# cassiusfive/balatro-gym

Hardware: AMD Instinct MI355X
Metric: env-steps/sec at 65536 envs, random policy; achieved HBM GB/s vs peak (higher is better)
Workload: dtype int64/f64

## Files before the change

### balatro_gym_amd/csrc/bg_device.h

```cpp
#pragma once
#include <hip/hip_runtime.h>
#include <stdint.h>
#include "bg_tables.h"

#define BG_NHOT 8
#define BG_NDECK 4
#define BG_NCOLD 7
#define BG_NTMPL 2
#define BG_MT_N 624
#define BG_MT_M 397
#define BG_MTS 640
#define BG_BLOCK 64

#define BG_DEVERR_GSTREAM 1u
#define BG_DEVERR_SHOPBLK 2u
#define BG_DEVERR_DECKRING 4u
#define BG_DEVERR_SHOPRING 8u

typedef __attribute__((address_space(1))) unsigned long long g_u64;
typedef __attribute__((address_space(1))) uint32_t g_u32;
__device__ __forceinline__ unsigned long long bg_ld8a(const void* p) { return __hip_atomic_load((g_u64*)p, __ATOMIC_RELAXED, __HIP_MEMORY_SCOPE_AGENT); }
__device__ __forceinline__ uint32_t bg_ld4a(const void* p) { return __hip_atomic_load((g_u32*)p, __ATOMIC_RELAXED, __HIP_MEMORY_SCOPE_AGENT); }
__device__ __forceinline__ void bg_st8a(void* p, unsigned long long v) { __hip_atomic_store((g_u64*)p, v, __ATOMIC_RELAXED, __HIP_MEMORY_SCOPE_AGENT); }
__device__ __forceinline__ uint4 bg_ld16a(const void* p) {
// ... 202 lines not shown
}
__device__ __forceinline__ Deck0 bg_load_deck0(const BgDev& d, int env) {
  uint4 c = d.deck[env];
  Deck0 r;
  r.lo = ((uint64_t)c.y << 32) | c.x;
  r.hi = ((uint64_t)c.w << 32) | c.z;
  return r;
}
__device__ __forceinline__ void bg_deck_set(Deck0& dk, int k, uint4 c) {
  if (k == 0) { dk.lo = ((uint64_t)c.y << 32) | c.x; dk.hi = ((uint64_t)c.w << 32) | c.z; }
}
__device__ __forceinline__ void bg_deck_set(DeckLds& dk, int k, uint4 c) {
  dk.col[(4 * k) * BG_RB] = c.x; dk.col[(4 * k + 1) * BG_RB] = c.y; dk.col[(4 * k + 2) * BG_RB] = c.z; dk.col[(4 * k + 3) * BG_RB] = c.w;
}
__device__ __forceinline__ int bg_card(const BgDev& d, int env, const Deck0& k, int idx) {
  if (idx < 16) return (int)(((idx < 8 ? k.lo : k.hi) >> (8 * (idx & 7))) & 0xffull);
  const uint32_t* p = (const uint32_t*)&d.deck[(size_t)(idx >> 4) * d.N + env];
  return (int)((bg_ld4a(p + ((idx & 15) >> 2)) >> (8 * (idx & 3))) & 0xffu);
}
template <int S, bool C> struct DeckLdsS { lds_u32* col; static constexpr bool kCards = C; };
template <int S, bool C>
__device__ __forceinline__ void bg_deck_set(DeckLdsS<S, C>& dk, int k, uint4 c) {
  dk.col[(4 * k) * S] = c.x; dk.col[(4 * k + 1) * S] = c.y; dk.col[(4 * k + 2) * S] = c.z; dk.col[(4 * k + 3) * S] = c.w;
}
template <int S, bool C>
__device__ __forceinline__ int bg_card(const BgDev& d, int env, const DeckLdsS<S, C>& k, int idx) {
  return (int)((const lds_u8*)k.col)[(idx >> 2) * (S * 4) + (idx & 3)];
}
__device__ __forceinline__ int bg_card(const BgDev& d, int env, const DeckLds& k, int idx) {
  return (int)((const lds_u8*)k.col)[(idx >> 2) * (BG_RB * 4) + (idx & 3)];
}

struct DeckHead { uint64_t lo, hi; };
__device__ __forceinline__ DeckHead bg_deck_head(const BgDev& d, int env, const Deck0& k) { return DeckHead{k.lo, k.hi}; }
template <int S, bool C>
__device__ __forceinline__ DeckHead bg_deck_head(const BgDev& d, int env, const DeckLdsS<S, C>& k) {
  const uint32_t a = k.col[0], b = k.col[S], c = k.col[2 * S], e = k.col[3 * S];
  return DeckHead{((uint64_t)b << 32) | a, ((uint64_t)e << 32) | c};
}
template <class DK>
__device__ __forceinline__ int bg_card_h(const BgDev& d, int env, const DK& k, const DeckHead& h, int idx) {
  if (idx < 16) return (int)(((idx < 8 ? h.lo : h.hi) >> (8 * (idx & 7))) & 0xffull);
  return bg_card(d, env, k, idx);
}

__device__ __forceinline__ uint32_t bg_temper(uint32_t y) {
  y ^= (y >> 11);
  y ^= (y << 7) & 0x9d2c5680u;
  y ^= (y << 15) & 0xefc60000u;
  y ^= (y >> 18);
  return y;
}
__device__ __forceinline__ uint32_t bg_twist(uint32_t a, uint32_t b, uint32_t far) {
  uint32_t y = (a & 0x80000000u) | (b & 0x7fffffffu);
  return far ^ (y >> 1) ^ ((y & 1u) ? 0x9908b0dfu : 0u);
}

// ... 300 lines not shown
```

### balatro_gym_amd/csrc/bg_engine3.h

```cpp
#pragma once

#ifdef BG_E3_TIMING
#define E3T_DECL() unsigned long long e3t_[8] = {0,0,0,0,0,0,0,0}, e3t0_ = __builtin_readcyclecounter()
#define E3T(k) do { const unsigned long long n_ = __builtin_readcyclecounter(); e3t_[k] += n_ - e3t0_; e3t0_ = n_; } while (0)
#define E3T_CNT(k, v) do { e3t_[k] += (v); } while (0)
#define E3T_FLUSH(base) do { if (lane == 0 && d.dbg) for (int k_ = 0; k_ < 8; k_++) atomicAdd(&d.dbg[(base) + k_], e3t_[k_]); } while (0)
constexpr bool kE3Timing = true, kE3Tl = true;
#else
#define E3T_DECL() const unsigned long long e3t_[8] = {0,0,0,0,0,0,0,0}; (void)e3t_
#define E3T(k) do {} while (0)
#define E3T_CNT(k, v) do {} while (0)
#define E3T_FLUSH(base) do {} while (0)
constexpr bool kE3Timing = false;
#ifdef BG_E3_TL
constexpr bool kE3Tl = true;
#else
constexpr bool kE3Tl = false;
#endif
#endif

#define BG_E3_REC_STORE(v, p) __builtin_nontemporal_store(v, p)
#define BG_E3_SPARSE 8u
#define BG_E3_SPARSE2 16u
#define BG_E3_ACTB 8
template <int NOW, int KS, int NSV>
struct E3Lds {
  static constexpr int NE = NOW * KS * BG_BLOCK;
  bg_u32x4 s_img[NE][22];
  uint4 s_c34[2][NE];
  unsigned long long s_mask[NE];
  uint32_t s_prod[NE];
  uint16_t s_ans[NE];
  uint32_t s_q[2][NE];
  __attribute__((aligned(16))) uint32_t s_ctl[8];
  uint32_t s_win[NSV][BG_WIN][BG_BLOCK];
  uint2 s_list[NOW][KS * BG_BLOCK];
  uint4 s_nd[BG_NDECK][NE];
  uint32_t s_ndst[NE];
  bg_u32x4 s_zero;
  unsigned long long s_stats[6];
  uint32_t s_owners_left;
  JTables jt;
};
template <bool HASH, bool CARDS, int NOW, int KS, int NSV, bool ACT = false>
__global__ __launch_bounds__((NOW + NSV) * BG_BLOCK, 2) void bg_engine3_kernel(BgDev d, EngineArgs a) {
  constexpr int NE = NOW * KS * BG_BLOCK, LNE = NE == 256 ? 8 : (NE == 128 ? 7 : 6);
  static_assert(NE == 64 || NE == 128 || NE == 256, "envs per workgroup (a request carries the env's lane in 8 bits)");
  __shared__ E3Lds<NOW, KS, NSV> L;
  auto& s_img = L.s_img; auto& s_c34 = L.s_c34; auto& s_mask = L.s_mask; auto& s_prod = L.s_prod; auto& s_ans = L.s_ans; auto& s_q = L.s_q;
  auto& s_ctl = L.s_ctl; auto& s_win = L.s_win; auto& s_list = L.s_list; auto& s_zero = L.s_zero; auto& s_owners_left = L.s_owners_left; auto& jt = L.jt;
  auto& s_nd = L.s_nd; auto& s_ndst = L.s_ndst;
  __shared__ int s_actb[ACT ? BG_E3_ACTB : 1][ACT ? NE : 1];
  __builtin_amdgcn_s_setprio(2);
  const unsigned long long e3_k0 = kE3Tl ? wall_clock64() : 0ull;
  BG_PROBE_INIT();
  bg_tables_load(&jt, d.jtab);
  const int tid = threadIdx.x, lane = tid & 63;
  const int wave = tid >> 6;
  const int epw = (NE == 64 && a.epw >= 1u && a.epw < 64u) ? (int)a.epw : NE;
  const int env0 = blockIdx.x * epw;
  const int n_live = d.N - env0 < epw ? d.N - env0 : epw;
  using DeckT = typename std::conditional<CARDS, Deck0C, Deck0>::type;
  const size_t N = (size_t)d.N;
  typedef __attribute__((address_space(3))) const char lds_cc;
  if (tid < 8) s_ctl[tid] = 0;
  if (tid == 0) { s_zero = bg_u32x4{0u, 0u, 0u, 0u}; s_owners_left = NOW; }
  if (tid < 6) L.s_stats[tid] = 0ull;
  for (int l = tid; l < NE; l += (NOW + NSV) * BG_BLOCK) {
    const int env = env0 + l;
    s_q[0][l] = 0; s_q[1][l] = 0; s_ans[l] = 0; s_ndst[l] = 0;
    if (l < n_live) {
      uint4 c[BG_NHOT];
#pragma unroll
      for (int k = 0; k < BG_NHOT; k++) c[k] = d.hot[(size_t)k * N + env];
      s_c34[0][l] = c[3]; s_c34[1][l] = c[4];
      DeckT dk; static_cast<Deck0&>(dk) = bg_load_deck0(d, env);
      const uint32_t prod = d.prod_view ? d.prod_view[env] : 0u;
      s_prod[l] = prod;
      Env e;
      bg_unpack(c, e);
      bg_derive_ready(e, prod);
      s_ndst[l] = e.d_ready > 0 ? 1u : 0u;
      if (e.d_ready > 0) {
#pragma unroll
        for (int k = 0; k < BG_NDECK; k++) s_nd[k][l] = d.ndeck[((size_t)e.d_head * BG_NDECK + k) * N + env];
      }
      ShopRegs sr; sr.valid = false;
      const uint64_t mask = bg_action_mask(d, env, e, sr);
      s_mask[l] = mask;
      const ObsPtrs none{};
      bg_write_obs_impl<false, 3>(d, env, 0, e, dk, none, mask, sr, RowExtra{0.0, 0, 0u}, RowStage{(lds_u4*)&s_img[l][0], nullptr});
    }
  }
  __syncthreads();
  if constexpr (kE3Timing) if (lane == 0) { uint32_t hw; asm volatile("s_getreg_b32 %0, hwreg(HW_REG_HW_ID)" : "=s"(hw)); atomicOr(&s_ctl[2], ((hw >> 4) & 3u) << (2 * wave)); }
  const unsigned long long e3_w0 = kE3Tl ? wall_clock64() : 0ull;
  if constexpr (kE3Tl) {
    if (tid == 0 && d.dbg) atomicAdd(&d.dbg[28], e3_w0 - e3_k0);
    __syncthreads();
  }
  const uint32_t T = (uint32_t)a.T;
  if (wave < NOW) {
    const uint32_t bmod3 = (uint32_t)(a.env_index0 % 3ull);
    lds_cc* const imgb = (lds_cc*)&s_img[0][0];
    const bool whole = a.obs.row_stride == 384u;
    uint32_t rsel[3], cmul[3], cib[3], cgl[3];
#pragma unroll
    for (int j = 0; j < 3; j++) {
      const uint32_t pidx = (uint32_t)j * BG_BLOCK + (uint32_t)lane, rs = (pidx * 2731u) >> 16, c = pidx - 24u * rs;
      rsel[j] = rs; cgl[j] = 16u * c;
      cmul[j] = c < 22u ? 16u * 22u : 0u;
      cib[j] = c < 22u ? 16u * c : (uint32_t)((lds_cc*)&s_zero - imgb);
    }
    uint32_t t[KS], nreq[KS];
    bool waiting[KS], terminal[KS];
    uint4 rc3[KS], rc4[KS];
    uint64_t rmask[KS];
    uint64_t px[KS];
    size_t prow[KS];
    int pblind[KS];
    uint32_t abase[KS];
    uint32_t athr[KS];
#pragma unroll
    for (int s = 0; s < KS; s++) {
      t[s] = 0; nreq[s] = 0; waiting[s] = false;
      const int l = (wave * KS + s) * BG_BLOCK + lane;
      if constexpr (ACT) {
        abase[s] = 0; athr[s] = 100u;
        prow[s] = (size_t)(env0 + l);
        if (l < n_live) {
          const uint32_t cap = (d.hot[(size_t)7 * N + (size_t)(env0 + l)].w >> 16) & 0xffu;
          if (cap > 0u && cap < 100u) athr[s] = cap;
        }
      } else {
        const int env = env0 + l;
        const uint64_t gi0 = a.env_index0 + (uint64_t)env;
        px[s] = a.policy_seed + 0x9E3779B97F4A7C15ull * (gi0 + 1) + BG_POLICY_PSI * (a.t0 + 1);
        prow[s] = (size_t)env;
        pblind[s] = a.policy == 2 ? 45 + (int)((bmod3 + (uint32_t)env % 3u) % 3u) : 45;
      }
      rc3[s] = s_c34[0][l]; rc4[s] = s_c34[1][l]; rmask[s] = s_mask[l];
      const lds_u32* im = (const lds_u32*)&s_img[l][0];
      terminal[s] = bg_b(rc3[s].x, 0) > (ACT ? athr[s] : 100u) || (int64_t)(((uint64_t)im[33] << 32) | im[32]) > 1000000000ll;
    }
    uint64_t n_steps = 0, rbits = 0, ohash = 0;
    uint32_t idle = 0, aiter = 0;
    E3T_DECL();
    for (;;) {
      bg_u32x4 ndv[KS][BG_NDECK];
      bool ndp[KS];
#pragma unroll
      for (int s = 0; s < KS; s++) ndp[s] = false;
      bool busy = false;
#pragma unroll
      for (int s = 0; s < KS; s++) busy = busy || ((wave * KS + s) * BG_BLOCK + lane < n_live && (t[s] < T || waiting[s]));
      if (__ballot(busy) == 0ull) break;
      E3T_CNT(4, 1);
      if constexpr (ACT) {
// ... 21 lines not shown
        const int l = (wave * KS + s) * BG_BLOCK + lane, env = env0 + l;
        const bool live = l < n_live;
        lds_u32* const img32 = (lds_u32*)&s_img[l][0];
        lds_u8* const img8 = (lds_u8*)&s_img[l][0];
        const size_t row = prow[s];
        bool fin = false;
        if (waiting[s] && bg_lds_ld(&s_ans[l]) == (nreq[s] & 0xffffu)) {
          waiting[s] = false; fin = true;
          const uint32_t nds = bg_lds_ld(&s_ndst[l]);
          if ((nds & 0xffu) == 2u) {
#pragma unroll
            for (int k = 0; k < BG_NDECK; k++) ndv[s][k] = *(const __attribute__((address_space(1))) bg_u32x4*)&d.ndeck[((size_t)(nds >> 8) * BG_NDECK + k) * N + env];
            bg_lds_st(&s_ndst[l], 0u);
            ndp[s] = true;
          }
          rc3[s] = s_c34[0][l]; rc4[s] = s_c34[1][l]; rmask[s] = s_mask[l];
          terminal[s] = bg_b(rc3[s].x, 0) > (ACT ? athr[s] : 100u) || (int64_t)(((uint64_t)img32[33] << 32) | img32[32]) > 1000000000ll;
        }
        else if (live && !waiting[s] && t[s] < T) {
          uint64_t mask = rmask[s];
          const uint4 c3 = rc3[s];
          const uint32_t phase = bg_b(c3.x, 2), discards_left = bg_b(c3.y, 0), nsel0 = bg_b(c3.y, 3);
          int action;
          if constexpr (ACT) action = s_actb[(t[s] - abase[s]) & (BG_E3_ACTB - 1u)][l];
          else {
            Env pe; pe.phase = (int)phase;
            PolicyLane pl; pl.seed_env = 0; pl.blind = pblind[s];
            action = bg_policy_action_fast(pe, mask, a.policy, pl, px[s], (lds_JTables*)&jt);
          }
          double reward = 0.0;
          const bool valid = action >= 0 && action < 60 && ((mask >> (action & 63)) & 1ull);
          const bool term = terminal[s];
          if (!term && valid && phase == 0u && action >= 2 && action < 10) {
            const int pos = action - 2;
            Env te; te.sel = ((uint64_t)rc4[s].w << 32) | rc4[s].z; te.nsel = (int)nsel0;
            bg_toggle_select(te, pos);
            rc4[s].z = (uint32_t)te.sel; rc4[s].w = (uint32_t)(te.sel >> 32);
            rc3[s].y = (rc3[s].y & 0x00ffffffu) | ((uint32_t)te.nsel << 24);
            *(lds_u64*)&img32[2 * pos] = te.nsel > (int)nsel0 ? 1ull : 0ull;
            if ((te.nsel > 0) != (nsel0 > 0u)) {
              const uint32_t play = te.nsel > 0 ? 1u : 0u, disc = (te.nsel > 0 && discards_left > 0u) ? 1u : 0u;
              mask = (mask & ~3ull) | play | ((uint64_t)disc << 1);
              rmask[s] = mask;
              *(__attribute__((address_space(3))) uint16_t*)&img8[BG_ROW_ACTION_MASK] = (uint16_t)(play | (disc << 8));
            }
            fin = true;
          } else if (!term && valid && phase == 1u && action == 31 && (int)(int8_t)bg_b(c3.y, 1) <= (int)bg_b(c3.y, 2)) {
            const uint32_t nhand = bg_b(c3.y, 2), ncons = bg_b(c3.z, 1);
            rc3[s].x &= 0xff00ffffu;
            uint64_t m = (((1ull << (nhand < 8u ? nhand : 8u)) - 1ull) << 2) | (((1ull << ncons) - 1ull) << 10);
            if (nsel0 > 0u) m |= 1ull | (discards_left > 0u ? 2ull : 0ull);
            mask = m;
            rmask[s] = mask;
#pragma unroll
            for (int wq = 0; wq < 15; wq++) img32[44 + wq] = __umul24((uint32_t)(mask >> (4 * wq)) & 0xfu, 0x204081u) & 0x01010101u;
#pragma unroll
            for (int wq = 64; wq < 74; wq++) img32[wq] = 0u;
            img8[BG_ROW_PHASE] = 0;
            fin = true;
          } else if (!term && !valid) { reward = -1.0; fin = true; }
          else {
            s_c34[0][l] = rc3[s]; s_c34[1][l] = rc4[s]; s_mask[l] = mask;
            if constexpr (ACT) img32[43] = (uint32_t)action;
            const int q = (!term && phase == 0u && action == 0) ? 0 : 1;
            const uint32_t slot = __hip_atomic_fetch_add(&s_ctl[q], 1u, __ATOMIC_RELAXED, __HIP_MEMORY_SCOPE_WORKGROUP);
            bg_lds_st(&s_q[q][slot & (NE - 1)], (uint32_t)l | (((slot >> LNE) & 0xffu) << 8) | (((uint32_t)action & 0x7fffu) << 16) | BG_ITEM_VALID);
            nreq[s]++;
            waiting[s] = true;
          }
          if (fin) {
            *(__attribute__((address_space(3))) double*)&img32[34] = reward;
            img32[43] = (uint32_t)action;
            img8[BG_ROW_TERMINATED] = 0;
          }
        }
        if (fin) {
          const uint64_t rb = ((uint64_t)img32[35] << 32) | img32[34];
          if (HASH) ohash ^= bg_hash_image((const lds_u4*)&s_img[l][0]) * (0x9E3779B97F4A7C15ull + 2 * (uint64_t)(a.t0 + t[s])) + (a.env_index0 + (uint64_t)env);
          n_steps++;
          rbits ^= rb * (2 * (uint64_t)(a.t0 + t[s]) + 1);
          t[s]++;
          if constexpr (!ACT) px[s] += BG_POLICY_PSI;
          if (a.obs_stride_steps) prow[s] += N;
        }
        const unsigned long long fms = __ballot(fin);
        const bool lastrec = fin && a.gworld != 0u && t[s] == T;
        if (fin) s_list[wave][nb + __builtin_amdgcn_mbcnt_hi((uint32_t)(fms >> 32), __builtin_amdgcn_mbcnt_lo((uint32_t)fms, 0u))] = make_uint2((uint32_t)row, (uint32_t)l | (lastrec ? 0x100u : 0u));
        nb += (uint32_t)__popcll(fms);
        glast = glast || lastrec;
      }
      E3T(0);
      if (nb) {
        idle = 0;
        BG_WAVE_SYNC();
        typedef uint32_t bg_u32x2 __attribute__((ext_vector_type(2)));
        lds_cc* const lsb = (lds_cc*)&s_list[wave][0];
#define BG_E3_LIVE(idx) ((idx) < nb)
#define BG_E3_ROW(x) (x)
#define BG_E3_COPY_GROUPS(NU, G0) do { \
          bg_u32x2 ce[NU][3]; \
          bg_u32x4 v[NU][3]; \
          _Pragma("unroll") for (int u = 0; u < NU; u++) _Pragma("unroll") for (int j = 0; j < 3; j++) \
            ce[u][j] = *(__attribute__((address_space(3))) const bg_u32x2*)(lsb + ((((G0) + 8u * (uint32_t)u + rsel[j]) & (KS * BG_BLOCK - 1u)) << 3)); \
          _Pragma("unroll") for (int u = 0; u < NU; u++) _Pragma("unroll") for (int j = 0; j < 3; j++) \
            v[u][j] = *(__attribute__((address_space(3))) const bg_u32x4*)(imgb + __umul24(ce[u][j].y & 0xffu, cmul[j]) + cib[j]); \
          _Pragma("unroll") for (int u = 0; u < NU; u++) _Pragma("unroll") for (int j = 0; j < 3; j++) \
            if (BG_E3_LIVE((G0) + 8u * (uint32_t)u + rsel[j])) \
              BG_E3_REC_STORE(v[u][j], (__attribute__((address_space(1))) bg_u32x4*)(a.obs.rows + ((size_t)BG_E3_ROW(ce[u][j].x) * 384u + cgl[j]))); \
        } while (0)
        const uint32_t nbs = (uint32_t)__builtin_amdgcn_readfirstlane((int)nb);
        if (whole && nbs <= BG_E3_SPARSE) {
          BG_E3_COPY_GROUPS(1, 0u);
        } else if (whole && nbs <= BG_E3_SPARSE2) {
          BG_E3_COPY_GROUPS(2, 0u);
        } else if (whole) {
          for (uint32_t g0 = 0; g0 < nb; g0 += 32u) BG_E3_COPY_GROUPS(4, g0);
        } else {
          const uint32_t total = 22u * nb;
          for (uint32_t q0 = (uint32_t)lane; q0 < total; q0 += 4u * BG_BLOCK) {
            bg_u32x2 ce[4]; uint32_t cpc[4]; bg_u32x4 v[4];
#pragma unroll
            for (int k = 0; k < 4; k++) {
              const uint32_t q = q0 + (uint32_t)k * BG_BLOCK, r = (q * 2979u) >> 16;
              cpc[k] = q - 22u * r;
              ce[k] = *(__attribute__((address_space(3))) const bg_u32x2*)(lsb + ((r < nb ? r : 0u) << 3));
            }
#pragma unroll
            for (int k = 0; k < 4; k++) v[k] = s_img[ce[k].y & 0xffu][cpc[k]];
#pragma unroll
            for (int k = 0; k < 4; k++)
              if (q0 + (uint32_t)k * BG_BLOCK < total)
                __builtin_nontemporal_store(v[k], (__attribute__((address_space(1))) bg_u32x4*)(a.obs.rows + (size_t)ce[k].x * (size_t)a.obs.row_stride + 16u * cpc[k]));
          }
        }
        if (a.gworld != 0u && __ballot(glast) != 0ull) {
          const uint32_t total = 22u * nb;
          for (uint32_t q = (uint32_t)lane; q < total; q += BG_BLOCK) {
            const uint32_t r = (q * 2979u) >> 16, pc = q - 22u * r;
            const bg_u32x2 ce = *(__attribute__((address_space(3))) const bg_u32x2*)(lsb + (r << 3));
            if (ce.y & 0x100u) {
              const uint32_t gl = ce.y & 0xffu;
              const bg_u32x4 v = s_img[gl][pc];
              const size_t off = ((size_t)a.grank * N + (size_t)(env0 + (int)gl)) * 352u + 16u * pc;
              for (uint32_t g = 0; g < a.gworld; g++) __builtin_nontemporal_store(v, (__attribute__((address_space(1))) bg_u32x4*)(a.gpeer[g] + off));
            }
          }
        }
        BG_WAVE_SYNC();
#pragma unroll
        for (int s = 0; s < KS; s++) {
          if (ndp[s]) {
            const int l = (wave * KS + s) * BG_BLOCK + lane;
#pragma unroll
            for (int k = 0; k < BG_NDECK; k++) *(__attribute__((address_space(3))) bg_u32x4*)&s_nd[k][l] = ndv[s][k];
            bg_lds_st(&s_ndst[l], 1u);
            ndp[s] = false;
          }
// ... 63 lines not shown
      {
        uint32_t got = 0;
        if ((uint32_t)lane < nb) item = bg_lds_ld(slotp);
        if (lane == 0) got = atomicCAS(&s_ctl[4 + cls], head, head + nb) == head ? 1u : 0u;
        if (__builtin_amdgcn_readfirstlane(got) == 0u) continue;
      }
      polls = 0;
      E3T(0);
      if ((uint32_t)lane < nb) {
        uint32_t spin = 0;
        const uint32_t want = BG_ITEM_VALID | ((((head + (uint32_t)lane) >> LNE) & 0xffu) << 8);
        while ((item & (BG_ITEM_VALID | 0xff00u)) != want && ++spin < BG_SPIN_LIMIT) { __builtin_amdgcn_s_sleep(1); item = bg_lds_ld(slotp); }
        if ((item & (BG_ITEM_VALID | 0xff00u)) != want) atomicOr(d.err, BG_DEVERR_SPIN);
        else {
          const int l = (int)(item & 0xffu), env = env0 + l;
          const int action = ACT ? (int)((const lds_u32*)&s_img[l][0])[43] : (int)((item >> 16) & 0x7fffu);
          uint64_t mask = s_mask[l];
          BG_PROBE_BEGIN();
          uint4 c[BG_NHOT];
#pragma unroll
          for (int k = 0; k < BG_NHOT; k++) if (k != 3 && k != 4) c[k] = d.hot[(size_t)k * N + env];
          c[3] = s_c34[0][l]; c[4] = s_c34[1][l];
          DeckT dk; static_cast<Deck0&>(dk) = bg_load_deck0(d, env);
          RngWin w;
          bg_win_init(w, &s_win[sidx][0][lane], &jt);
          Env e;
          bg_unpack(c, e);
          BG_PROBE(23);
          bg_derive_ready(e, s_prod[l]);
          ShopRegs sr; sr.valid = false;
          StepOut o;
          bg_step_init(o);
          o.bd_dst = nullptr;
          if (bg_step_guards(e, mask, action, o)) bg_env_dispatch(d, env, e, w, sr, dk, action, o);
          BG_PROBE(cls == 0 ? 20 : 21);
          if (e.max_ante > 0 && e.ante > e.max_ante) { o.terminated = true; o.flags |= 256; }
          if (o.terminated) n_eps++;
          if (o.terminated && a.autoreset) {
            const bool have = bg_lds_ld(&s_ndst[l]) == 1u;
            bg_env_reset(d, env, e, dk, nullptr, have ? (lds_cu4*)&s_nd[0][l] : (lds_cu4*)nullptr, NE);
            bg_lds_st(&s_ndst[l], e.d_ready > 0 ? (2u | ((uint32_t)e.d_head << 8)) : 0u);
          }
          if constexpr (CARDS) bg_vm_drain();
          BG_PROBE(24);
          mask = bg_action_mask(d, env, e, sr);
          BG_PROBE(25);
          const ObsPtrs none{};
          bg_write_obs_impl<false, 3>(d, env, 0, e, dk, none, mask, sr, RowExtra{o.reward, action, o.terminated ? 1u : 0u}, RowStage{(lds_u4*)&s_img[l][0], nullptr});
          BG_PROBE(26);
          bg_pack(e, c);
#pragma unroll
          for (int k = 0; k < BG_NHOT; k++) if (k != 3 && k != 4) d.hot[(size_t)k * N + env] = c[k];
          s_c34[0][l] = c[3]; s_c34[1][l] = c[4];
          s_mask[l] = mask;
          if (o.hand_type >= 0) { n_plays++; ssum += o.final_score; }
          bg_lds_st(&s_ans[l], bg_lds_ld(&s_ans[l]) + 1u);
          BG_PROBE(27);
        }
      }
      E3T(1 + cls); E3T_CNT(4 + cls, 1); E3T_CNT(6 + cls, nb);
    }
    E3T_FLUSH(8);
    if constexpr (kE3Tl) if (lane == 0 && d.dbg) atomicAdd(&d.dbg[30], wall_clock64() - e3_k0);
    if (a.stats) bg_stats_wave(L.s_stats, 0, n_eps, n_plays, ssum, 0, 0);
  }
  BG_PROBE_FLUSH(d);
  __syncthreads();
  for (int l = tid; l < n_live; l += (NOW + NSV) * BG_BLOCK) {
    d.hot[(size_t)3 * N + env0 + l] = s_c34[0][l];
    d.hot[(size_t)4 * N + env0 + l] = s_c34[1][l];
  }
  if (a.stats) bg_stats_flush(a.stats, L.s_stats, tid);
  if constexpr (kE3Tl) if (tid == 0 && d.dbg) atomicAdd(&d.dbg[31], wall_clock64() - e3_k0);
}
```

### balatro_gym_amd/csrc/bg_step.h

```cpp
#pragma once
#include "bg_device.h"

struct StepOut {
  double reward;
  int64_t final_score;
  double terms[8];
  int32_t error, flags, aux;
  int32_t hand_type, cards_played;
  bool terminated;
  double* bd_dst;
};

struct ShopRegs { uint4 c3, c4, c5, c6; bool valid; };
__device__ __forceinline__ void bg_shop_load(const BgDev& d, int env, ShopRegs& sr) {
  if (sr.valid) return;
  size_t N = d.N;
  sr.c3 = bg_ld16a(&d.cold[3 * N + env]); sr.c4 = bg_ld16a(&d.cold[4 * N + env]); sr.c5 = bg_ld16a(&d.cold[5 * N + env]); sr.c6 = bg_ld16a(&d.cold[6 * N + env]);
  sr.valid = true;
}
__device__ __forceinline__ void bg_shop_store(const BgDev& d, int env, const ShopRegs& sr) {
  size_t N = d.N;
  d.cold[3 * N + env] = sr.c3; d.cold[4 * N + env] = sr.c4; d.cold[5 * N + env] = sr.c5; d.cold[6 * N + env] = sr.c6;
}
__device__ __forceinline__ void bg_shop_unpack(const ShopRegs& sr, int32_t cost[9], uint32_t tp[9]) {
// ... 1261 lines not shown
__device__ __forceinline__ uint32_t bg_obs_selm(const Env& e) {
  uint32_t selm = 0;
#pragma unroll 1
  for (int i = 0; i < e.nsel; i++) selm |= 1u << bg_get8(e.sel, i);
  return selm;
}
__device__ __forceinline__ float bg_obs_prf(const Env& e) {
  int64_t need1 = e.chips_needed > 1 ? e.chips_needed : 1;
  double pr = (double)e.round_chips / (double)need1;
  return (float)(pr < 2.0 ? pr : 2.0);
}
typedef uint32_t bg_u32x4 __attribute__((ext_vector_type(4)));
typedef __attribute__((address_space(3))) bg_u32x4 lds_u4;
typedef __attribute__((address_space(3))) unsigned long long lds_u64;
#define BG_STAGE_NP 11
struct RowStage { lds_u4* stage; lds_u64* addr; };
#define BG_WAVE_SYNC() __builtin_amdgcn_wave_barrier()

typedef __attribute__((address_space(3))) unsigned long long lds_stat;
__device__ __forceinline__ void bg_stats_wave(unsigned long long* st, uint64_t n_steps, uint64_t n_eps, uint64_t n_plays, int64_t ssum, uint64_t rbits, uint64_t ohash) {
#pragma unroll
  for (int off = 32; off > 0; off >>= 1) {
    n_steps += __shfl_down(n_steps, off); n_eps += __shfl_down(n_eps, off); n_plays += __shfl_down(n_plays, off);
    ssum += __shfl_down(ssum, off); rbits ^= __shfl_down(rbits, off); ohash ^= __shfl_down(ohash, off);
  }
  if ((threadIdx.x & 63u) == 0u) {
    lds_stat* s = (lds_stat*)st;
    if (n_steps) __hip_atomic_fetch_add(&s[0], (unsigned long long)n_steps, __ATOMIC_RELAXED, __HIP_MEMORY_SCOPE_WORKGROUP);
    if (n_eps) __hip_atomic_fetch_add(&s[1], (unsigned long long)n_eps, __ATOMIC_RELAXED, __HIP_MEMORY_SCOPE_WORKGROUP);
    if (n_plays) __hip_atomic_fetch_add(&s[2], (unsigned long long)n_plays, __ATOMIC_RELAXED, __HIP_MEMORY_SCOPE_WORKGROUP);
    if (ssum) __hip_atomic_fetch_add(&s[3], (unsigned long long)ssum, __ATOMIC_RELAXED, __HIP_MEMORY_SCOPE_WORKGROUP);
// ... 62 lines not shown
    a = (a | (a << 8)) & 0x00ff00ffu; a = (a | (a << 4)) & 0x0f0f0f0fu;
    b = (b | (b << 8)) & 0x00ff00ffu; b = (b | (b << 4)) & 0x0f0f0f0fu;
    lv[w] = a + b;
    BG_MIX(lv[w]);
  }
  BG_MIX(mask);
  uint32_t mq[15];
#pragma unroll
  for (int w = 0; w < 15; w++) {
    const uint32_t bits = (uint32_t)(mask >> (4 * w)) & 0xfu;
    mq[w] = __umul24(bits, 0x204081u) & 0x01010101u;
  }
  BG_MIX(((uint64_t)(uint32_t)e.hp_total << 32) | (uint32_t)e.best_hand);
  BG_MIX(e.boss_type);
#undef BG_MIX
  if (p.rows || STAGE == 3) {
    uint32_t w[88];
#pragma unroll
    for (int i = 0; i < 8; i++) { w[2 * i] = (selm >> i) & 1u; w[2 * i + 1] = 0u; }
#pragma unroll
    for (int i = 0; i < 8; i++) { w[16 + 2 * i] = (e.face_down >> i) & 1u; w[17 + 2 * i] = 0u; }
    w[32] = (uint32_t)(uint64_t)e.chips_scored; w[33] = (uint32_t)((uint64_t)e.chips_scored >> 32);
    { const uint64_t rb = (uint64_t)__double_as_longlong(rx.reward); w[34] = (uint32_t)rb; w[35] = (uint32_t)(rb >> 32); }
    w[36] = (uint32_t)(int32_t)e.round_chips; w[37] = __float_as_uint(prf); w[38] = 1u; w[39] = (uint32_t)e.chips_needed;
    w[40] = (uint32_t)e.money; w[41] = (uint32_t)e.hp_total; w[42] = (uint32_t)(int32_t)e.best_hand; w[43] = (uint32_t)rx.action;
#pragma unroll
    for (int i = 0; i < 15; i++) w[44 + i] = mq[i];
#pragma unroll
    for (int i = 0; i < 5; i++) { w[59 + i] = jq[i]; w[64 + i] = it[i]; w[69 + i] = co[i]; }
    w[74] = cq; w[75] = 0u;
    w[76] = ((uint32_t)e.ante & 0xffffu) << 16;
    w[77] = ((uint32_t)e.shop_reroll_state & 0xffffu) | ((uint32_t)(handb & 0xffffull) << 16);
    w[78] = (uint32_t)(handb >> 16);
    w[79] = (uint32_t)(handb >> 48) | ((lv[0] & 0xffffu) << 16);
    w[80] = (lv[0] >> 16) | (lv[1] << 16);
    w[81] = (lv[1] >> 16) | (lv[2] << 16);
    w[82] = (lv[2] >> 16) | (((uint32_t)e.nhand & 0xffu) << 16) | ((uint32_t)(52 - e.ndrop + e.nfo) << 24);
    w[83] = ((uint32_t)e.round & 0xffu) | (((uint32_t)e.hands_left & 0xffu) << 8) | (((uint32_t)e.discards_left & 0xffu) << 16) |
            (((uint32_t)e.njokers & 0xffu) << 24);
    w[84] = 5u | (((uint32_t)e.ncons & 0xffu) << 8) | (2u << 16) | (((uint32_t)e.phase & 0xffu) << 24);
    w[85] = (e.boss_type ? 1u : 0u) | (((uint32_t)e.boss_type & 0xffu) << 8) | ((rx.terminated & 1u) << 16);
    w[86] = 0u; w[87] = 0u;
    uint8_t* rowp = p.rows + row * (size_t)p.row_stride;
    if constexpr (STAGE == 3) {
#pragma unroll
      for (int k = 0; k < 22; k++) rs.stage[k] = bg_u32x4{w[4 * k], w[4 * k + 1], w[4 * k + 2], w[4 * k + 3]};
    } else if constexpr (STAGE == 2) {
      const unsigned long long act = __ballot(1);
      const uint32_t A = (uint32_t)__popcll(act);
      const uint32_t rank = __builtin_amdgcn_mbcnt_hi((uint32_t)(act >> 32), __builtin_amdgcn_mbcnt_lo((uint32_t)act, 0u));
      rs.addr[rank] = (unsigned long long)rowp;
#pragma unroll
      for (int sl = 0; sl < 3; sl++) {
        const int np = sl == 0 ? 8 : 7, base = sl == 0 ? 0 : (sl == 1 ? 8 : 15);
#pragma unroll
        for (int c = 0; c < np; c++) { const int k = base + c; rs.stage[rank * np + c] = bg_u32x4{w[4 * k], w[4 * k + 1], w[4 * k + 2], w[4 * k + 3]}; }
        BG_WAVE_SYNC();
#pragma unroll
        for (int k = 0; k < np; k++) {
// ... 135 lines not shown
#pragma unroll
    for (int i = 0; i < 12; i++) q[i] = (int8_t)b[318 + i]; }
  if (p.hand_size) p.hand_size[row] = (int8_t)b[330];
  if (p.deck_size) p.deck_size[row] = (int8_t)b[331];
  if (p.round) p.round[row] = (int8_t)b[332];
  if (p.hands_left) p.hands_left[row] = (int8_t)b[333];
  if (p.discards_left) p.discards_left[row] = (int8_t)b[334];
  if (p.joker_count) p.joker_count[row] = (int8_t)b[335];
  if (p.joker_slots) p.joker_slots[row] = (int8_t)b[336];
  if (p.consumable_count) p.consumable_count[row] = (int8_t)b[337];
  if (p.consumable_slots) p.consumable_slots[row] = (int8_t)b[338];
  if (p.phase) p.phase[row] = (int8_t)b[339];
  if (p.boss_blind_active) p.boss_blind_active[row] = (int8_t)b[340];
  if (p.boss_blind_type) p.boss_blind_type[row] = (int8_t)b[341];
}
__device__ __forceinline__ uint64_t bg_hash_image(const lds_u4* img) {
  uint64_t h = 0x9E3779B97F4A7C15ull;
#pragma unroll
  for (int k = 0; k < 22; k++) {
    bg_u32x4 v = img[k];
    if (k == 8) { v.z = 0; v.w = 0; }
    if (k == 10) v.w = 0;
    if (k == 21) v.y &= 0xff00ffffu;
    h ^= ((uint64_t)v.y << 32) | v.x; h *= 0xBF58476D1CE4E5B9ull; h ^= h >> 29;
    h ^= ((uint64_t)v.w << 32) | v.z; h *= 0x94D049BB133111EBull; h ^= h >> 31;
  }
  return h;
}

struct PolicyLane { uint64_t seed_env; int blind; };
__device__ __forceinline__ PolicyLane bg_policy_lane(int policy, uint64_t policy_seed, uint64_t env_index) {
  PolicyLane p;
  p.seed_env = policy_seed + 0x9E3779B97F4A7C15ull * (env_index + 1);
  p.blind = policy == 2 ? 45 + (int)(env_index % 3) : 45;
  return p;
}
__device__ __forceinline__ int bg_policy_action(const Env& e, uint64_t mask, int policy, const PolicyLane& pl, uint64_t t) {
  if (policy != 0) {
    if (e.phase == 2) return pl.blind;
    if (e.phase == 1) return 31;
  }
  const int nv = __popcll(mask);
// ... 68 lines not shown
```

Measured before the change: 7.352 billion.

## Keep hot env state in LDS and compact staged obs image flags

```diff
diff --git a/balatro_gym_amd/csrc/bg_device.h b/balatro_gym_amd/csrc/bg_device.h
--- a/balatro_gym_amd/csrc/bg_device.h
+++ b/balatro_gym_amd/csrc/bg_device.h
@@ -240,7 +240,8 @@
   dk.col[(4 * k) * BG_RB] = c.x; dk.col[(4 * k + 1) * BG_RB] = c.y; dk.col[(4 * k + 2) * BG_RB] = c.z; dk.col[(4 * k + 3) * BG_RB] = c.w;
 }
 __device__ __forceinline__ int bg_card(const BgDev& d, int env, const Deck0& k, int idx) {
-  if (idx < 16) return (int)(((idx < 8 ? k.lo : k.hi) >> (8 * (idx & 7))) & 0xffull);
+  const uint64_t lo = k.lo, hi = k.hi;
+  if (idx < 16) return (int)(((idx < 8 ? lo : hi) >> (8 * (idx & 7))) & 0xffull);
   const uint32_t* p = (const uint32_t*)&d.deck[(size_t)(idx >> 4) * d.N + env];
   return (int)((bg_ld4a(p + ((idx & 15) >> 2)) >> (8 * (idx & 3))) & 0xffu);
 }
@@ -266,7 +267,8 @@
 }
 template <class DK>
 __device__ __forceinline__ int bg_card_h(const BgDev& d, int env, const DK& k, const DeckHead& h, int idx) {
-  if (idx < 16) return (int)(((idx < 8 ? h.lo : h.hi) >> (8 * (idx & 7))) & 0xffull);
+  const uint64_t lo = h.lo, hi = h.hi;
+  if (idx < 16) return (int)(((idx < 8 ? lo : hi) >> (8 * (idx & 7))) & 0xffull);
   return bg_card(d, env, k, idx);
 }
 
diff --git a/balatro_gym_amd/csrc/bg_engine3.h b/balatro_gym_amd/csrc/bg_engine3.h
--- a/balatro_gym_amd/csrc/bg_engine3.h
+++ b/balatro_gym_amd/csrc/bg_engine3.h
@@ -23,13 +23,24 @@
 #define BG_E3_SPARSE 8u
 #define BG_E3_SPARSE2 16u
 #define BG_E3_ACTB 8
+#define BG_E3_IB(row_byte) ((row_byte) - BG_IMG_B0)
+#define BG_E3_IW(row_byte) (BG_E3_IB(row_byte) / 4)
+#define BG_E3_LY_LANE 0xffu
+#define BG_E3_LY_LAST 0x100u
+#define BG_E3_LY_FLAGS 16u
+#define BG_E3_LY_DEAD 9u
+static_assert(((BG_E3_LY_LANE | BG_E3_LY_LAST | (0xffffu << BG_E3_LY_FLAGS)) & (3u << BG_E3_LY_DEAD)) == 0u, "the dead bits of a list entry's .y are in use");
+static_assert(BG_ROW_CHIPS_SCORED == BG_IMG_B0, "the compact image starts at the first record byte behind the flag arrays");
 template <int NOW, int KS, int NSV>
 struct E3Lds {
   static constexpr int NE = NOW * KS * BG_BLOCK;
-  bg_u32x4 s_img[NE][22];
+  bg_u32x4 s_img[NE][BG_IMG_NP];
   uint4 s_c34[2][NE];
+  uint4 s_hot[BG_NHOT - 2][NE];
+  static constexpr int hot_row(int k) { return k < 3 ? k : k - 2; }
   unsigned long long s_mask[NE];
   uint32_t s_prod[NE];
+  uint16_t s_flag[NE];
   uint16_t s_ans[NE];
   uint32_t s_q[2][NE];
   __attribute__((aligned(16))) uint32_t s_ctl[8];
@@ -49,7 +60,8 @@
   __shared__ E3Lds<NOW, KS, NSV> L;
   auto& s_img = L.s_img; auto& s_c34 = L.s_c34; auto& s_mask = L.s_mask; auto& s_prod = L.s_prod; auto& s_ans = L.s_ans; auto& s_q = L.s_q;
   auto& s_ctl = L.s_ctl; auto& s_win = L.s_win; auto& s_list = L.s_list; auto& s_zero = L.s_zero; auto& s_owners_left = L.s_owners_left; auto& jt = L.jt;
-  auto& s_nd = L.s_nd; auto& s_ndst = L.s_ndst;
+  auto& s_nd = L.s_nd; auto& s_ndst = L.s_ndst; auto& s_flag = L.s_flag; auto& s_hot = L.s_hot;
+  using LdsT = E3Lds<NOW, KS, NSV>;
   __shared__ int s_actb[ACT ? BG_E3_ACTB : 1][ACT ? NE : 1];
   __builtin_amdgcn_s_setprio(2);
   const unsigned long long e3_k0 = kE3Tl ? wall_clock64() : 0ull;
@@ -74,6 +86,8 @@
 #pragma unroll
       for (int k = 0; k < BG_NHOT; k++) c[k] = d.hot[(size_t)k * N + env];
       s_c34[0][l] = c[3]; s_c34[1][l] = c[4];
+#pragma unroll
+      for (int k = 0; k < BG_NHOT; k++) if (k != 3 && k != 4) s_hot[LdsT::hot_row(k)][l] = c[k];
       DeckT dk; static_cast<Deck0&>(dk) = bg_load_deck0(d, env);
       const uint32_t prod = d.prod_view ? d.prod_view[env] : 0u;
       s_prod[l] = prod;
@@ -89,7 +103,7 @@
       const uint64_t mask = bg_action_mask(d, env, e, sr);
       s_mask[l] = mask;
       const ObsPtrs none{};
-      bg_write_obs_impl<false, 3>(d, env, 0, e, dk, none, mask, sr, RowExtra{0.0, 0, 0u}, RowStage{(lds_u4*)&s_img[l][0], nullptr});
+      bg_write_obs_impl<false, 4>(d, env, 0, e, dk, none, mask, sr, RowExtra{0.0, 0, 0u}, RowStage{(lds_u4*)&s_img[l][0], nullptr, (lds_u16*)&s_flag[l]});
     }
   }
   __syncthreads();
@@ -104,18 +118,21 @@
     const uint32_t bmod3 = (uint32_t)(a.env_index0 % 3ull);
     lds_cc* const imgb = (lds_cc*)&s_img[0][0];
     const bool whole = a.obs.row_stride == 384u;
-    uint32_t rsel[3], cmul[3], cib[3], cgl[3];
+    uint32_t rsel[3], cmul[3], cib[3], cgl[3], cfs[3];
 #pragma unroll
     for (int j = 0; j < 3; j++) {
       const uint32_t pidx = (uint32_t)j * BG_BLOCK + (uint32_t)lane, rs = (pidx * 2731u) >> 16, c = pidx - 24u * rs;
+      const bool inimg = c >= (uint32_t)BG_IMG_P0 && c < 22u;
       rsel[j] = rs; cgl[j] = 16u * c;
-      cmul[j] = c < 22u ? 16u * 22u : 0u;
-      cib[j] = c < 22u ? 16u * c : (uint32_t)((lds_cc*)&s_zero - imgb);
+      cmul[j] = inimg ? 16u * BG_IMG_NP : 0u;
+      cib[j] = inimg ? 16u * (c - (uint32_t)BG_IMG_P0) : (uint32_t)((lds_cc*)&s_zero - imgb);
+      cfs[j] = c < (uint32_t)BG_IMG_P0 ? BG_E3_LY_FLAGS + 2u * c : BG_E3_LY_DEAD;
     }
     uint32_t t[KS], nreq[KS];
     bool waiting[KS], terminal[KS];
     uint4 rc3[KS], rc4[KS];
     uint64_t rmask[KS];
+    uint32_t rflag[KS];
     uint64_t px[KS];
     size_t prow[KS];
     int pblind[KS];
@@ -129,7 +146,7 @@
         abase[s] = 0; athr[s] = 100u;
         prow[s] = (size_t)(env0 + l);
         if (l < n_live) {
-          const uint32_t cap = (d.hot[(size_t)7 * N + (size_t)(env0 + l)].w >> 16) & 0xffu;
+          const uint32_t cap = (s_hot[LdsT::hot_row(7)][l].w >> 16) & 0xffu;
           if (cap > 0u && cap < 100u) athr[s] = cap;
         }
       } else {
@@ -139,9 +156,9 @@
         prow[s] = (size_t)env;
         pblind[s] = a.policy == 2 ? 45 + (int)((bmod3 + (uint32_t)env % 3u) % 3u) : 45;
       }
-      rc3[s] = s_c34[0][l]; rc4[s] = s_c34[1][l]; rmask[s] = s_mask[l];
+      rc3[s] = s_c34[0][l]; rc4[s] = s_c34[1][l]; rmask[s] = s_mask[l]; rflag[s] = s_flag[l];
       const lds_u32* im = (const lds_u32*)&s_img[l][0];
-      terminal[s] = bg_b(rc3[s].x, 0) > (ACT ? athr[s] : 100u) || (int64_t)(((uint64_t)im[33] << 32) | im[32]) > 1000000000ll;
+      terminal[s] = bg_b(rc3[s].x, 0) > (ACT ? athr[s] : 100u) || (int64_t)(((uint64_t)im[BG_E3_IW(BG_ROW_CHIPS_SCORED) + 1] << 32) | im[BG_E3_IW(BG_ROW_CHIPS_SCORED)]) > 1000000000ll;
     }
     uint64_t n_steps = 0, rbits = 0, ohash = 0;
     uint32_t idle = 0, aiter = 0;
@@ -193,8 +210,8 @@
             bg_lds_st(&s_ndst[l], 0u);
             ndp[s] = true;
           }
-          rc3[s] = s_c34[0][l]; rc4[s] = s_c34[1][l]; rmask[s] = s_mask[l];
-          terminal[s] = bg_b(rc3[s].x, 0) > (ACT ? athr[s] : 100u) || (int64_t)(((uint64_t)img32[33] << 32) | img32[32]) > 1000000000ll;
+          rc3[s] = s_c34[0][l]; rc4[s] = s_c34[1][l]; rmask[s] = s_mask[l]; rflag[s] = s_flag[l];
+          terminal[s] = bg_b(rc3[s].x, 0) > (ACT ? athr[s] : 100u) || (int64_t)(((uint64_t)img32[BG_E3_IW(BG_ROW_CHIPS_SCORED) + 1] << 32) | img32[BG_E3_IW(BG_ROW_CHIPS_SCORED)]) > 1000000000ll;
         }
         else if (live && !waiting[s] && t[s] < T) {
           uint64_t mask = rmask[s];
@@ -216,12 +233,12 @@
             bg_toggle_select(te, pos);
             rc4[s].z = (uint32_t)te.sel; rc4[s].w = (uint32_t)(te.sel >> 32);
             rc3[s].y = (rc3[s].y & 0x00ffffffu) | ((uint32_t)te.nsel << 24);
-            *(lds_u64*)&img32[2 * pos] = te.nsel > (int)nsel0 ? 1ull : 0ull;
+            rflag[s] = bg_flag_toggle(rflag[s], pos, te.nsel > (int)nsel0);
             if ((te.nsel > 0) != (nsel0 > 0u)) {
               const uint32_t play = te.nsel > 0 ? 1u : 0u, disc = (te.nsel > 0 && discards_left > 0u) ? 1u : 0u;
               mask = (mask & ~3ull) | play | ((uint64_t)disc << 1);
               rmask[s] = mask;
-              *(__attribute__((address_space(3))) uint16_t*)&img8[BG_ROW_ACTION_MASK] = (uint16_t)(play | (disc << 8));
+              *(__attribute__((address_space(3))) uint16_t*)&img8[BG_E3_IB(BG_ROW_ACTION_MASK)] = (uint16_t)(play | (disc << 8));
             }
             fin = true;
           } else if (!term && valid && phase == 1u && action == 31 && (int)(int8_t)bg_b(c3.y, 1) <= (int)bg_b(c3.y, 2)) {
@@ -232,15 +249,15 @@
             mask = m;
             rmask[s] = mask;
 #pragma unroll
-            for (int wq = 0; wq < 15; wq++) img32[44 + wq] = __umul24((uint32_t)(mask >> (4 * wq)) & 0xfu, 0x204081u) & 0x01010101u;
-#pragma unroll
-            for (int wq = 64; wq < 74; wq++) img32[wq] = 0u;
-            img8[BG_ROW_PHASE] = 0;
+            for (int wq = 0; wq < 15; wq++) img32[BG_E3_IW(BG_ROW_ACTION_MASK) + wq] = __umul24((uint32_t)(mask >> (4 * wq)) & 0xfu, 0x204081u) & 0x01010101u;
+#pragma unroll
+            for (int wq = 0; wq < 10; wq++) img32[BG_E3_IW(BG_ROW_SHOP_ITEMS) + wq] = 0u;
+            img8[BG_E3_IB(BG_ROW_PHASE)] = 0;
             fin = true;
           } else if (!term && !valid) { reward = -1.0; fin = true; }
           else {
             s_c34[0][l] = rc3[s]; s_c34[1][l] = rc4[s]; s_mask[l] = mask;
-            if constexpr (ACT) img32[43] = (uint32_t)action;
+            if constexpr (ACT) img32[BG_E3_IW(BG_ROW_ACTION)] = (uint32_t)action;
             const int q = (!term && phase == 0u && action == 0) ? 0 : 1;
             const uint32_t slot = __hip_atomic_fetch_add(&s_ctl[q], 1u, __ATOMIC_RELAXED, __HIP_MEMORY_SCOPE_WORKGROUP);
             bg_lds_st(&s_q[q][slot & (NE - 1)], (uint32_t)l | (((slot >> LNE) & 0xffu) << 8) | (((uint32_t)action & 0x7fffu) << 16) | BG_ITEM_VALID);
@@ -248,14 +265,14 @@
             waiting[s] = true;
           }
           if (fin) {
-            *(__attribute__((address_space(3))) double*)&img32[34] = reward;
-            img32[43] = (uint32_t)action;
-            img8[BG_ROW_TERMINATED] = 0;
+            *(__attribute__((address_space(3))) double*)&img32[BG_E3_IW(BG_ROW_REWARD)] = reward;
+            img32[BG_E3_IW(BG_ROW_ACTION)] = (uint32_t)action;
+            img8[BG_E3_IB(BG_ROW_TERMINATED)] = 0;
           }
         }
         if (fin) {
-          const uint64_t rb = ((uint64_t)img32[35] << 32) | img32[34];
-          if (HASH) ohash ^= bg_hash_image((const lds_u4*)&s_img[l][0]) * (0x9E3779B97F4A7C15ull + 2 * (uint64_t)(a.t0 + t[s])) + (a.env_index0 + (uint64_t)env);
+          const uint64_t rb = ((uint64_t)img32[BG_E3_IW(BG_ROW_REWARD) + 1] << 32) | img32[BG_E3_IW(BG_ROW_REWARD)];
+          if (HASH) ohash ^= bg_hash_image_compact((const lds_u4*)&s_img[l][0], rflag[s]) * (0x9E3779B97F4A7C15ull + 2 * (uint64_t)(a.t0 + t[s])) + (a.env_index0 + (uint64_t)env);
           n_steps++;
           rbits ^= rb * (2 * (uint64_t)(a.t0 + t[s]) + 1);
           t[s]++;
@@ -264,7 +281,7 @@
         }
         const unsigned long long fms = __ballot(fin);
         const bool lastrec = fin && a.gworld != 0u && t[s] == T;
-        if (fin) s_list[wave][nb + __builtin_amdgcn_mbcnt_hi((uint32_t)(fms >> 32), __builtin_amdgcn_mbcnt_lo((uint32_t)fms, 0u))] = make_uint2((uint32_t)row, (uint32_t)l | (lastrec ? 0x100u : 0u));
+        if (fin) s_list[wave][nb + __builtin_amdgcn_mbcnt_hi((uint32_t)(fms >> 32), __builtin_amdgcn_mbcnt_lo((uint32_t)fms, 0u))] = make_uint2((uint32_t)row, (uint32_t)l | (lastrec ? BG_E3_LY_LAST : 0u) | (rflag[s] << BG_E3_LY_FLAGS));
         nb += (uint32_t)__popcll(fms);
         glast = glast || lastrec;
       }
@@ -282,7 +299,9 @@
           _Pragma("unroll") for (int u = 0; u < NU; u++) _Pragma("unroll") for (int j = 0; j < 3; j++) \
             ce[u][j] = *(__attribute__((address_space(3))) const bg_u32x2*)(lsb + ((((G0) + 8u * (uint32_t)u + rsel[j]) & (KS * BG_BLOCK - 1u)) << 3)); \
           _Pragma("unroll") for (int u = 0; u < NU; u++) _Pragma("unroll") for (int j = 0; j < 3; j++) \
-            v[u][j] = *(__attribute__((address_space(3))) const bg_u32x4*)(imgb + __umul24(ce[u][j].y & 0xffu, cmul[j]) + cib[j]); \
+            v[u][j] = *(__attribute__((address_space(3))) const bg_u32x4*)(imgb + __umul24(ce[u][j].y & BG_E3_LY_LANE, cmul[j]) + cib[j]); \
+          _Pragma("unroll") for (int u = 0; u < NU; u++) _Pragma("unroll") for (int j = 0; j < 3; j++) { \
+            v[u][j].x |= (ce[u][j].y >> cfs[j]) & 1u; v[u][j].z |= (ce[u][j].y >> (cfs[j] + 1u)) & 1u; } \
           _Pragma("unroll") for (int u = 0; u < NU; u++) _Pragma("unroll") for (int j = 0; j < 3; j++) \
             if (BG_E3_LIVE((G0) + 8u * (uint32_t)u + rsel[j])) \
               BG_E3_REC_STORE(v[u][j], (__attribute__((address_space(1))) bg_u32x4*)(a.obs.rows + ((size_t)BG_E3_ROW(ce[u][j].x) * 384u + cgl[j]))); \
@@ -305,7 +324,7 @@
               ce[k] = *(__attribute__((address_space(3))) const bg_u32x2*)(lsb + ((r < nb ? r : 0u) << 3));
             }
 #pragma unroll
-            for (int k = 0; k < 4; k++) v[k] = s_img[ce[k].y & 0xffu][cpc[k]];
+            for (int k = 0; k < 4; k++) v[k] = bg_img_piece(&s_img[ce[k].y & BG_E3_LY_LANE][0], ce[k].y >> BG_E3_LY_FLAGS, cpc[k]);
 #pragma unroll
             for (int k = 0; k < 4; k++)
               if (q0 + (uint32_t)k * BG_BLOCK < total)
@@ -317,9 +336,9 @@
           for (uint32_t q = (uint32_t)lane; q < total; q += BG_BLOCK) {
             const uint32_t r = (q * 2979u) >> 16, pc = q - 22u * r;
             const bg_u32x2 ce = *(__attribute__((address_space(3))) const bg_u32x2*)(lsb + (r << 3));
-            if (ce.y & 0x100u) {
-              const uint32_t gl = ce.y & 0xffu;
-              const bg_u32x4 v = s_img[gl][pc];
+            if (ce.y & BG_E3_LY_LAST) {
+              const uint32_t gl = ce.y & BG_E3_LY_LANE;
+              const bg_u32x4 v = bg_img_piece(&s_img[gl][0], ce.y >> BG_E3_LY_FLAGS, pc);
               const size_t off = ((size_t)a.grank * N + (size_t)(env0 + (int)gl)) * 352u + 16u * pc;
               for (uint32_t g = 0; g < a.gworld; g++) __builtin_nontemporal_store(v, (__attribute__((address_space(1))) bg_u32x4*)(a.gpeer[g] + off));
             }
@@ -413,12 +432,12 @@
         if ((item & (BG_ITEM_VALID | 0xff00u)) != want) atomicOr(d.err, BG_DEVERR_SPIN);
         else {
           const int l = (int)(item & 0xffu), env = env0 + l;
-          const int action = ACT ? (int)((const lds_u32*)&s_img[l][0])[43] : (int)((item >> 16) & 0x7fffu);
+          const int action = ACT ? (int)((const lds_u32*)&s_img[l][0])[BG_E3_IW(BG_ROW_ACTION)] : (int)((item >> 16) & 0x7fffu);
           uint64_t mask = s_mask[l];
           BG_PROBE_BEGIN();
           uint4 c[BG_NHOT];
 #pragma unroll
-          for (int k = 0; k < BG_NHOT; k++) if (k != 3 && k != 4) c[k] = d.hot[(size_t)k * N + env];
+          for (int k = 0; k < BG_NHOT; k++) if (k != 3 && k != 4) c[k] = s_hot[LdsT::hot_row(k)][l];
           c[3] = s_c34[0][l]; c[4] = s_c34[1][l];
           DeckT dk; static_cast<Deck0&>(dk) = bg_load_deck0(d, env);
           RngWin w;
@@ -445,11 +464,11 @@
           mask = bg_action_mask(d, env, e, sr);
           BG_PROBE(25);
           const ObsPtrs none{};
-          bg_write_obs_impl<false, 3>(d, env, 0, e, dk, none, mask, sr, RowExtra{o.reward, action, o.terminated ? 1u : 0u}, RowStage{(lds_u4*)&s_img[l][0], nullptr});
+          bg_write_obs_impl<false, 4>(d, env, 0, e, dk, none, mask, sr, RowExtra{o.reward, action, o.terminated ? 1u : 0u}, RowStage{(lds_u4*)&s_img[l][0], nullptr, (lds_u16*)&s_flag[l]});
           BG_PROBE(26);
           bg_pack(e, c);
 #pragma unroll
-          for (int k = 0; k < BG_NHOT; k++) if (k != 3 && k != 4) d.hot[(size_t)k * N + env] = c[k];
+          for (int k = 0; k < BG_NHOT; k++) if (k != 3 && k != 4) s_hot[LdsT::hot_row(k)][l] = c[k];
           s_c34[0][l] = c[3]; s_c34[1][l] = c[4];
           s_mask[l] = mask;
           if (o.hand_type >= 0) { n_plays++; ssum += o.final_score; }
@@ -466,8 +485,8 @@
   BG_PROBE_FLUSH(d);
   __syncthreads();
   for (int l = tid; l < n_live; l += (NOW + NSV) * BG_BLOCK) {
-    d.hot[(size_t)3 * N + env0 + l] = s_c34[0][l];
-    d.hot[(size_t)4 * N + env0 + l] = s_c34[1][l];
+#pragma unroll
+    for (int k = 0; k < BG_NHOT; k++) d.hot[(size_t)k * N + env0 + l] = (k == 3 || k == 4) ? s_c34[k - 3][l] : s_hot[LdsT::hot_row(k)][l];
   }
   if (a.stats) bg_stats_flush(a.stats, L.s_stats, tid);
   if constexpr (kE3Tl) if (tid == 0 && d.dbg) atomicAdd(&d.dbg[31], wall_clock64() - e3_k0);
diff --git a/balatro_gym_amd/csrc/bg_step.h b/balatro_gym_amd/csrc/bg_step.h
--- a/balatro_gym_amd/csrc/bg_step.h
+++ b/balatro_gym_amd/csrc/bg_step.h
@@ -1299,7 +1299,19 @@
 typedef __attribute__((address_space(3))) bg_u32x4 lds_u4;
 typedef __attribute__((address_space(3))) unsigned long long lds_u64;
 #define BG_STAGE_NP 11
-struct RowStage { lds_u4* stage; lds_u64* addr; };
+typedef __attribute__((address_space(3))) uint16_t lds_u16;
+struct RowStage { lds_u4* stage; lds_u64* addr; lds_u16* flags = nullptr; };
+#define BG_IMG_W0 32
+#define BG_IMG_B0 (4 * BG_IMG_W0)
+#define BG_IMG_P0 (BG_IMG_W0 / 4)
+#define BG_IMG_NP (22 - BG_IMG_P0)
+__host__ __device__ __forceinline__ uint32_t bg_flag_bits(uint32_t selm, uint32_t face_down) { return (selm & 0xffu) | ((face_down & 0xffu) << 8); }
+__host__ __device__ __forceinline__ bg_u32x4 bg_flag_piece(uint32_t bits, uint32_t c) { return bg_u32x4{(bits >> (2u * c)) & 1u, 0u, (bits >> (2u * c + 1u)) & 1u, 0u}; }
+template <class P>
+__device__ __forceinline__ bg_u32x4 bg_img_piece(P img, uint32_t bits, uint32_t pc) {
+  return pc < (uint32_t)BG_IMG_P0 ? bg_flag_piece(bits, pc) : img[pc - (uint32_t)BG_IMG_P0];
+}
+__host__ __device__ __forceinline__ uint32_t bg_flag_toggle(uint32_t bits, int pos, bool joined) { return joined ? bits | (1u << pos) : bits & ~(1u << pos); }
 #define BG_WAVE_SYNC() __builtin_amdgcn_wave_barrier()
 
 typedef __attribute__((address_space(3))) unsigned long long lds_stat;
@@ -1392,35 +1404,43 @@
   BG_MIX(((uint64_t)(uint32_t)e.hp_total << 32) | (uint32_t)e.best_hand);
   BG_MIX(e.boss_type);
 #undef BG_MIX
-  if (p.rows || STAGE == 3) {
-    uint32_t w[88];
-#pragma unroll
-    for (int i = 0; i < 8; i++) { w[2 * i] = (selm >> i) & 1u; w[2 * i + 1] = 0u; }
-#pragma unroll
-    for (int i = 0; i < 8; i++) { w[16 + 2 * i] = (e.face_down >> i) & 1u; w[17 + 2 * i] = 0u; }
-    w[32] = (uint32_t)(uint64_t)e.chips_scored; w[33] = (uint32_t)((uint64_t)e.chips_scored >> 32);
-    { const uint64_t rb = (uint64_t)__double_as_longlong(rx.reward); w[34] = (uint32_t)rb; w[35] = (uint32_t)(rb >> 32); }
-    w[36] = (uint32_t)(int32_t)e.round_chips; w[37] = __float_as_uint(prf); w[38] = 1u; w[39] = (uint32_t)e.chips_needed;
-    w[40] = (uint32_t)e.money; w[41] = (uint32_t)e.hp_total; w[42] = (uint32_t)(int32_t)e.best_hand; w[43] = (uint32_t)rx.action;
-#pragma unroll
-    for (int i = 0; i < 15; i++) w[44 + i] = mq[i];
-#pragma unroll
-    for (int i = 0; i < 5; i++) { w[59 + i] = jq[i]; w[64 + i] = it[i]; w[69 + i] = co[i]; }
-    w[74] = cq; w[75] = 0u;
-    w[76] = ((uint32_t)e.ante & 0xffffu) << 16;
-    w[77] = ((uint32_t)e.shop_reroll_state & 0xffffu) | ((uint32_t)(handb & 0xffffull) << 16);
-    w[78] = (uint32_t)(handb >> 16);
-    w[79] = (uint32_t)(handb >> 48) | ((lv[0] & 0xffffu) << 16);
-    w[80] = (lv[0] >> 16) | (lv[1] << 16);
-    w[81] = (lv[1] >> 16) | (lv[2] << 16);
-    w[82] = (lv[2] >> 16) | (((uint32_t)e.nhand & 0xffu) << 16) | ((uint32_t)(52 - e.ndrop + e.nfo) << 24);
-    w[83] = ((uint32_t)e.round & 0xffu) | (((uint32_t)e.hands_left & 0xffu) << 8) | (((uint32_t)e.discards_left & 0xffu) << 16) |
+  if (p.rows || STAGE >= 3) {
+    constexpr int W0 = STAGE == 4 ? BG_IMG_W0 : 0;
+    uint32_t w[88 - W0];
+    if constexpr (STAGE != 4) {
+#pragma unroll
+      for (int i = 0; i < 8; i++) { w[2 * i] = (selm >> i) & 1u; w[2 * i + 1] = 0u; }
+#pragma unroll
+      for (int i = 0; i < 8; i++) { w[16 + 2 * i] = (e.face_down >> i) & 1u; w[17 + 2 * i] = 0u; }
+    }
+    w[32 - W0] = (uint32_t)(uint64_t)e.chips_scored; w[33 - W0] = (uint32_t)((uint64_t)e.chips_scored >> 32);
+    { const uint64_t rb = (uint64_t)__double_as_longlong(rx.reward); w[34 - W0] = (uint32_t)rb; w[35 - W0] = (uint32_t)(rb >> 32); }
+    w[36 - W0] = (uint32_t)(int32_t)e.round_chips; w[37 - W0] = __float_as_uint(prf); w[38 - W0] = 1u; w[39 - W0] = (uint32_t)e.chips_needed;
+    w[40 - W0] = (uint32_t)e.money; w[41 - W0] = (uint32_t)e.hp_total; w[42 - W0] = (uint32_t)(int32_t)e.best_hand; w[43 - W0] = (uint32_t)rx.action;
+#pragma unroll
+    for (int i = 0; i < 15; i++) w[44 - W0 + i] = mq[i];
+#pragma unroll
+    for (int i = 0; i < 5; i++) { w[59 - W0 + i] = jq[i]; w[64 - W0 + i] = it[i]; w[69 - W0 + i] = co[i]; }
+    w[74 - W0] = cq; w[75 - W0] = 0u;
+    w[76 - W0] = ((uint32_t)e.ante & 0xffffu) << 16;
+    w[77 - W0] = ((uint32_t)e.shop_reroll_state & 0xffffu) | ((uint32_t)(handb & 0xffffull) << 16);
+    w[78 - W0] = (uint32_t)(handb >> 16);
+    w[79 - W0] = (uint32_t)(handb >> 48) | ((lv[0] & 0xffffu) << 16);
+    w[80 - W0] = (lv[0] >> 16) | (lv[1] << 16);
+    w[81 - W0] = (lv[1] >> 16) | (lv[2] << 16);
+    w[82 - W0] = (lv[2] >> 16) | (((uint32_t)e.nhand & 0xffu) << 16) | ((uint32_t)(52 - e.ndrop + e.nfo) << 24);
+    w[83 - W0] = ((uint32_t)e.round & 0xffu) | (((uint32_t)e.hands_left & 0xffu) << 8) | (((uint32_t)e.discards_left & 0xffu) << 16) |
             (((uint32_t)e.njokers & 0xffu) << 24);
-    w[84] = 5u | (((uint32_t)e.ncons & 0xffu) << 8) | (2u << 16) | (((uint32_t)e.phase & 0xffu) << 24);
-    w[85] = (e.boss_type ? 1u : 0u) | (((uint32_t)e.boss_type & 0xffu) << 8) | ((rx.terminated & 1u) << 16);
-    w[86] = 0u; w[87] = 0u;
+    w[84 - W0] = 5u | (((uint32_t)e.ncons & 0xffu) << 8) | (2u << 16) | (((uint32_t)e.phase & 0xffu) << 24);
+    w[85 - W0] = (e.boss_type ? 1u : 0u) | (((uint32_t)e.boss_type & 0xffu) << 8) | ((rx.terminated & 1u) << 16);
+    w[86 - W0] = 0u; w[87 - W0] = 0u;
     uint8_t* rowp = p.rows + row * (size_t)p.row_stride;
-    if constexpr (STAGE == 3) {
+    if constexpr (STAGE == 4) {
+#pragma unroll
+      for (int k = 0; k < BG_IMG_NP; k++) rs.stage[k] = bg_u32x4{w[4 * k], w[4 * k + 1], w[4 * k + 2], w[4 * k + 3]};
+      *rs.flags = (uint16_t)bg_flag_bits(selm, (uint32_t)e.face_down);
+      return hsh;
+    } else if constexpr (STAGE == 3) {
 #pragma unroll
       for (int k = 0; k < 22; k++) rs.stage[k] = bg_u32x4{w[4 * k], w[4 * k + 1], w[4 * k + 2], w[4 * k + 3]};
     } else if constexpr (STAGE == 2) {
@@ -1586,11 +1606,12 @@
   if (p.boss_blind_active) p.boss_blind_active[row] = (int8_t)b[340];
   if (p.boss_blind_type) p.boss_blind_type[row] = (int8_t)b[341];
 }
-__device__ __forceinline__ uint64_t bg_hash_image(const lds_u4* img) {
+template <class F>
+__device__ __forceinline__ uint64_t bg_hash_pieces(F piece) {
   uint64_t h = 0x9E3779B97F4A7C15ull;
 #pragma unroll
   for (int k = 0; k < 22; k++) {
-    bg_u32x4 v = img[k];
+    bg_u32x4 v = piece(k);
     if (k == 8) { v.z = 0; v.w = 0; }
     if (k == 10) v.w = 0;
     if (k == 21) v.y &= 0xff00ffffu;
@@ -1598,6 +1619,10 @@
     h ^= ((uint64_t)v.w << 32) | v.z; h *= 0x94D049BB133111EBull; h ^= h >> 31;
   }
   return h;
+}
+__device__ __forceinline__ uint64_t bg_hash_image(const lds_u4* img) { return bg_hash_pieces([&](int k) { return img[k]; }); }
+__device__ __forceinline__ uint64_t bg_hash_image_compact(const lds_u4* img, uint32_t bits) {
+  return bg_hash_pieces([&](int k) { return bg_img_piece(img, bits, (uint32_t)k); });
 }
 
 struct PolicyLane { uint64_t seed_env; int blind; };
```

Result: faster. 7.542 billion (median of 6 runs) (+2.6%).
